# cristian-jfv/lattice-boltzmann-method

Hardware: AMD Instinct MI355X
Metric: MLUPS (million lattice updates/sec), D2Q9 BGK periodic box, f64 (higher is better)
Workload: dtype f64

## Files before the change

### lattice-boltzmann-method_amd/csrc/d2q9.hpp

```cpp
#pragma once
#include <type_traits>
#include <hip/hip_runtime.h>

#include "../../include/lbm_hip.h"

namespace lbm {

constexpr int Q = 9;

#define LBM_W0 (4.0 / 9.0)
#define LBM_WS (1.0 / 9.0)
#define LBM_WD (1.0 / 36.0)

__device__ __forceinline__ constexpr double wq(int q) {
  return q == 0 ? LBM_W0 : (q < 5 ? LBM_WS : LBM_WD);
}
__host__ __device__ __forceinline__ constexpr int icx(int q) {
  return (q == 1 || q == 5 || q == 8) ? 1 : ((q == 3 || q == 6 || q == 7) ? -1 : 0);
}
__host__ __device__ __forceinline__ constexpr int icy(int q) {
  return (q == 2 || q == 5 || q == 6) ? 1 : ((q == 4 || q == 7 || q == 8) ? -1 : 0);
}
__host__ __device__ __forceinline__ constexpr int opp(int q) {
  return q == 0 ? 0 : (q == 1 ? 3 : (q == 2 ? 4 : (q == 3 ? 1 : (q == 4 ? 2 : (q == 5 ? 7 : (q == 6 ? 8 : (q == 7 ? 5 : 6)))))));
// ... 349 lines not shown
    int row_end, int tiles_per_row, double* __restrict__ rho_out, double* __restrict__ u_out) {
  const long items = (long)(row_end - row_begin) * tiles_per_row;
  for (long it = blockIdx.x; it < items; it += gridDim.x) {
    const int r = row_begin + (int)(it / tiles_per_row);
    const int c = (int)(it % tiles_per_row) * 256 + threadIdx.x;
    if (c >= g.C) continue;
    const long rows[3] = {g.at(wrap_row(g, r + 1), 0), g.at(r, 0), g.at(wrap_row(g, r - 1), 0)};
    const int cols[3] = {wrap_col(g, c + 1), c, wrap_col(g, c - 1)};
    double f[Q];
#pragma unroll
    for (int q = 0; q < Q; ++q) {
      const double* src = po + q * g.plane + rows[icx(q) + 1] + cols[icy(q) + 1];
      f[q] = NT_LOAD ? __builtin_nontemporal_load(src) : *src;
    }
    double rho, ux, uy;
    m.collide(f, rho, ux, uy);
#pragma unroll
    for (int q = 0; q < Q; ++q) {
      double* dst = pn + q * g.plane + rows[1] + c;
      if (NT_STORE) __builtin_nontemporal_store(f[q], dst);
      else *dst = f[q];
    }
    if (WITH_MOMENTS) {
      const long o = (long)r * g.C + c, n = (long)g.R * g.C;
      rho_out[o] = rho;
      u_out[o] = ux;
      u_out[n + o] = uy;
    }
  }
}

template <class Model, int BLOCK, int ROWS, bool NT_LOAD, bool NT_STORE>
__global__ __launch_bounds__(BLOCK) void k_stream_collide_v3(
    double* __restrict__ pn, const double* __restrict__ po, Geom g, Model m, int row_begin,
    int row_end, int tiles_x, int n_items, int swizzle) {
  int item = blockIdx.x;
  if (swizzle) {
    const int chunk = (n_items + 7) >> 3;
    item = (item & 7) * chunk + (item >> 3);
    if (item >= n_items) return;
  }
  const int c = (item % tiles_x) * BLOCK + threadIdx.x;
  const int rbase = row_begin + (item / tiles_x) * ROWS;
  if (c >= g.C) return;
  const int cols[3] = {wrap_col(g, c + 1), c, wrap_col(g, c - 1)};
  double f[ROWS][Q];
#pragma unroll
  for (int k = 0; k < ROWS; ++k) {
    const int r = rbase + k;
    if (r < row_end) {
      const long rows[3] = {g.at(wrap_row(g, r + 1), 0), g.at(r, 0), g.at(wrap_row(g, r - 1), 0)};
#pragma unroll
      for (int q = 0; q < Q; ++q) {
        const double* src = po + q * g.plane + rows[icx(q) + 1] + cols[icy(q) + 1];
        f[k][q] = NT_LOAD ? __builtin_nontemporal_load(src) : *src;
      }
    }
  }
#pragma unroll
  for (int k = 0; k < ROWS; ++k) {
    const int r = rbase + k;
    if (r < row_end) {
      double rho, ux, uy;
      m.collide(f[k], rho, ux, uy);
      const long o = g.at(r, c);
#pragma unroll
      for (int q = 0; q < Q; ++q) {
        double* dst = pn + q * g.plane + o;
        if (NT_STORE) __builtin_nontemporal_store(f[k][q], dst);
        else *dst = f[k][q];
      }
    }
  }
}

template <class Model, int TR, int BLOCK, bool NT_STORE>
__global__ __launch_bounds__(BLOCK) void k_stream_collide_tb2(
    double* __restrict__ pn, const double* __restrict__ po, Geom g, Model m, int row_begin,
    int row_end, int tiles_x, int tiles_y, int order) {
  constexpr int TC = 64, LR = TR + 2, LC = TC + 2;
  __shared__ double s[Q][LR][LC];
  int tx, ty;
  if (order == 1) {
    const int xcd = blockIdx.x & 7, j = blockIdx.x >> 3;
    tx = (j / tiles_y) * 8 + xcd;
    ty = j % tiles_y;
  } else {
    tx = blockIdx.x % tiles_x;
    ty = blockIdx.x / tiles_x;
  }
  const int r0 = row_begin + ty * TR, c0 = tx * TC;
  for (int i = threadIdx.x; i < LR * LC; i += BLOCK) {
    const int lr = i / LC, lc = i - lr * LC;
    const int r = wrap_row(g, r0 + lr - 1), c = wrap_col(g, c0 + lc - 1);
    const long rows[3] = {g.at(wrap_row(g, r + 1), 0), g.at(r, 0), g.at(wrap_row(g, r - 1), 0)};
    const int cols[3] = {wrap_col(g, c + 1), c, wrap_col(g, c - 1)};
    double f[Q];
#pragma unroll
    for (int q = 0; q < Q; ++q) f[q] = po[q * g.plane + rows[icx(q) + 1] + cols[icy(q) + 1]];
    double rho, ux, uy;
    m.collide(f, rho, ux, uy);
#pragma unroll
    for (int q = 0; q < Q; ++q) s[q][lr][lc] = f[q];
  }
  __syncthreads();
  for (int i = threadIdx.x; i < TR * TC; i += BLOCK) {
    const int tr = i / TC, tc = i % TC;
    const int r = r0 + tr;
    if (r >= row_end) break;
    double f[Q];
#pragma unroll
    for (int q = 0; q < Q; ++q) f[q] = s[q][tr + 1 - icx(q)][tc + 1 - icy(q)];
    double rho, ux, uy;
    m.collide(f, rho, ux, uy);
    const long o = g.at(r, c0 + tc);
#pragma unroll
    for (int q = 0; q < Q; ++q) {
      double* dst = pn + q * g.plane + o;
      if (NT_STORE) __builtin_nontemporal_store(f[q], dst);
      else *dst = f[q];
    }
  }
}

#ifndef LBM_SW_DPP
#define LBM_SW_DPP 1
#endif
__device__ __forceinline__ double lane_from_prev(double v) {
#if LBM_SW_DPP
  int lo = __double2loint(v), hi = __double2hiint(v);
  lo = __builtin_amdgcn_update_dpp(lo, lo, 0x138, 0xf, 0xf, false);
  hi = __builtin_amdgcn_update_dpp(hi, hi, 0x138, 0xf, 0xf, false);
  return __hiloint2double(hi, lo);
#else
  return __shfl_up(v, 1);
#endif
}
__device__ __forceinline__ double lane_from_next(double v) {
#if LBM_SW_DPP
  int lo = __double2loint(v), hi = __double2hiint(v);
  lo = __builtin_amdgcn_update_dpp(lo, lo, 0x130, 0xf, 0xf, false);
  hi = __builtin_amdgcn_update_dpp(hi, hi, 0x130, 0xf, 0xf, false);
  return __hiloint2double(hi, lo);
#else
  return __shfl_down(v, 1);
#endif
}

constexpr int SW_LDS_LANES = 66;
__host__ __device__ constexpr int sw_lds_level_doubles() { return 12 * SW_LDS_LANES; }
__host__ __device__ constexpr int sw_lds_ring_doubles(int D) { return (D > 1 ? D - 1 : 1) * sw_lds_level_doubles(); }
__host__ __device__ constexpr int sw_grp_pos(int q) { return (q == 3 || q == 0 || q == 1) ? 0 : ((q == 6 || q == 2 || q == 5) ? 1 : 2); }

template <class Model, int D, int K, bool NT_STORE, bool HAS_BC = false, bool LDSR = false>
__device__ __forceinline__ void sw_iteration(double (&ring)[D > 1 ? D - 1 : 1][3][Q], double (&cur)[Q],
                                             double* __restrict__ pn, const double* __restrict__ po,
                                             const Geom& g, const Model& m, int i, int rbase, int R0,
                                             int R1, int c_load, const int (&cols)[3], bool lane_ok,
                                             int c_out, const Bc& bc = Bc{}, int c_raw = 0, double* lds = nullptr, int lane = 0) {
  double nxt[Q];
  {
    const int r1n = rbase + i + 1;
    int rr[3] = {r1n + 1, r1n, r1n - 1};
#pragma unroll
    for (int k = 0; k < 3; ++k) {
      if (g.ghost) rr[k] = rr[k] < -g.ghost ? -g.ghost : (rr[k] > g.R + g.ghost - 1 ? g.R + g.ghost - 1 : rr[k]);
      else rr[k] = rr[k] < 0 ? rr[k] + g.R : (rr[k] >= g.R ? rr[k] - g.R : rr[k]);
    }
#pragma unroll
    for (int q = 0; q < Q; ++q) {
      const char* rowp = reinterpret_cast<const char*>(po + q * g.plane + g.at(rr[icx(q) + 1], 0));
      nxt[q] = *reinterpret_cast<const double*>(rowp + (unsigned)cols[icy(q) + 1] * 8u);
    }
  }
  double f[Q], rho, ux, uy;
#pragma unroll
  for (int q = 0; q < Q; ++q) f[q] = cur[q];
  const bool col_in = c_raw >= 0 && c_raw < g.C;
  const bool wall_col = HAS_BC && col_in && ((c_raw == 0 && bc_is_wall(bc.col_lo)) || (c_raw == g.C - 1 && bc_is_wall(bc.col_hi)));
  const bool rows_wrap = HAS_BC && !g.ghost && !bc_is_wall(bc.row_lo) && !bc_is_wall(bc.row_hi);
  const int row_min = (HAS_BC && g.ghost && bc.row_lo == LBM_EDGE_HALO) ? -g.ghost : 0;
  const int row_max = (HAS_BC && g.ghost && bc.row_hi == LBM_EDGE_HALO) ? g.R + g.ghost - 1 : g.R - 1;
  if (HAS_BC) {
    int r1 = rbase + i;
    if (rows_wrap) r1 = r1 < 0 ? r1 + g.R : (r1 >= g.R ? r1 - g.R : r1);
    const bool wall_row = (r1 == 0 && bc_is_wall(bc.row_lo)) || (r1 == g.R - 1 && bc_is_wall(bc.row_hi));
    if (col_in && r1 >= row_min && r1 <= row_max && (wall_row || wall_col)) gather_walls(f, po, g, bc, r1, c_raw);
  }
  m.collide(f, rho, ux, uy);
#pragma unroll
  for (int l = 2; l <= D; ++l) {
    if constexpr (LDSR) {
      double* lv = lds + (l - 2) * sw_lds_level_doubles();
      double* slotA = lv;
      double* slotB = lv + 3 * SW_LDS_LANES;
      double* slotC = lv + (6 + 3 * (i & 1)) * SW_LDS_LANES;
      double fn[Q];
#pragma unroll
      for (int q = 0; q < Q; ++q) {
        if (icx(q) == 0) fn[q] = slotB[sw_grp_pos(q) * SW_LDS_LANES + lane + 1 - icy(q)];
        else if (icx(q) == 1) fn[q] = slotC[sw_grp_pos(q) * SW_LDS_LANES + lane + 1 - icy(q)];
      }
      __builtin_amdgcn_fence(__ATOMIC_RELEASE, "wavefront");
      __builtin_amdgcn_wave_barrier();
#pragma unroll
      for (int q = 0; q < Q; ++q) {
        double* dst = icx(q) == -1 ? slotA : (icx(q) == 0 ? slotB : slotC);
        dst[sw_grp_pos(q) * SW_LDS_LANES + lane + 1] = f[q];
      }
      __builtin_amdgcn_fence(__ATOMIC_RELEASE, "wavefront");
      __builtin_amdgcn_wave_barrier();
      __builtin_amdgcn_fence(__ATOMIC_ACQUIRE, "wavefront");
#pragma unroll
      for (int q = 0; q < Q; ++q)
        if (icx(q) == -1) fn[q] = slotA[sw_grp_pos(q) * SW_LDS_LANES + lane + 1 - icy(q)];
#pragma unroll
      for (int q = 0; q < Q; ++q) f[q] = fn[q];
    } else {
#pragma unroll
    for (int q = 0; q < Q; ++q) ring[l - 2][K][q] = f[q];
#pragma unroll
    for (int q = 0; q < Q; ++q) {
      const int slot = icx(q) == -1 ? K : (icx(q) == 0 ? (K + 2) % 3 : (K + 1) % 3);
      double v = ring[l - 2][slot][q];
      if (icy(q) == 1) v = lane_from_prev(v);
      else if (icy(q) == -1) v = lane_from_next(v);
      f[q] = v;
    }
    }
    if (HAS_BC && !LDSR) {
      int rl = rbase + i - (l - 1);
      if (rows_wrap) rl = rl < 0 ? rl + g.R : (rl >= g.R ? rl - g.R : rl);
      const bool wall_row = (rl == 0 && bc_is_wall(bc.row_lo)) || (rl == g.R - 1 && bc_is_wall(bc.row_hi));
      if (col_in && rl >= row_min && rl <= row_max && (wall_row || wall_col)) {
        double own[Q];
#pragma unroll
        for (int q = 0; q < Q; ++q) own[q] = ring[l - 2][(K + 2) % 3][q];
        bc_fixups_own(f, own, g, bc, rl, c_raw);
      }
    }
    m.collide(f, rho, ux, uy);
  }
  const int rD = rbase + i - (D - 1);
  if (lane_ok && rD >= R0 && rD < R1) {
    const long o = g.at(rD, 0);
#pragma unroll
    for (int q = 0; q < Q; ++q) {
      double* dst = reinterpret_cast<double*>(reinterpret_cast<char*>(pn + q * g.plane + o) + (unsigned)c_out * 8u);
      if (NT_STORE) __builtin_nontemporal_store(f[q], dst);
      else *dst = f[q];
    }
  }
#pragma unroll
  for (int q = 0; q < Q; ++q) cur[q] = nxt[q];
  (void)c_load;
}

#ifdef LBM_EXPERIMENTS
#include "experiments/sw_prefetch2.hpp"
#endif

__host__ __device__ constexpr int sw_strip_width(int D, bool full = false) {
  return full ? 64 - 2 * (D - 1) : (64 - 2 * (D - 1)) / 8 * 8;
}
template <class M, class = void>
struct sw_full_strips : std::false_type {};
template <class M>
struct sw_full_strips<M, std::void_t<decltype(M::kFullStrips)>> : std::bool_constant<M::kFullStrips> {};
__host__ __device__ constexpr int sw_waves_per_simd(int D) { return D <= 2 ? 4 : (D == 3 ? 3 : (D <= 5 ? 2 : 1)); }
template <class Model, int D, bool NT_STORE, bool HAS_BC, bool PF2, bool LDSR = false>
__device__ __forceinline__ void sw_wave_body(double* __restrict__ pn, const double* __restrict__ po, const Geom& g,
                                             const Model& m, int row_begin, int row_end, int rows_per_chunk, int strips,
                                             int wave, int lane, const Bc& bc, int strip0, int chunk_stride,
                                             double* lds = nullptr) {
  static_assert(!(LDSR && (HAS_BC || PF2)), "the LDS ring exists for the plain window only");
  constexpr int W = sw_strip_width(D, sw_full_strips<Model>::value);
  const int strip = strip0 + wave % strips, chunk = wave / strips;
  const int R0 = row_begin + chunk * (chunk_stride > 0 ? chunk_stride : rows_per_chunk);
  const int R1 = R0 + rows_per_chunk < row_end ? R0 + rows_per_chunk : row_end;
  int c = strip * W - (D - 1) + lane;
  const int c_raw = c;
  const bool lane_ok = lane >= D - 1 && lane < D - 1 + W && c < g.C;
  const bool walled_cols = HAS_BC && (bc_is_wall(bc.col_lo) || bc_is_wall(bc.col_hi));
  if (walled_cols) {
    c = c < 0 ? 0 : (c > g.C - 1 ? g.C - 1 : c);
  } else {
    c = c < 0 ? c + g.C : (c >= g.C ? c - g.C : c);
    c = c >= g.C ? c - g.C : c;
  }
  const int cols[3] = {walled_cols ? (c + 1 > g.C - 1 ? g.C - 1 : c + 1) : wrap_col(g, c + 1), c,
                       walled_cols ? (c - 1 < 0 ? 0 : c - 1) : wrap_col(g, c - 1)};
  const int rbase = R0 - (D - 1);
  const int n_iter = (R1 - R0) + 2 * (D - 1);
  double ring[D > 1 ? D - 1 : 1][3][Q];
#pragma unroll
  for (int a = 0; a < (D > 1 ? D - 1 : 1); ++a)
#pragma unroll
    for (int b = 0; b < 3; ++b)
#pragma unroll
      for (int q = 0; q < Q; ++q) ring[a][b][q] = 1.0;
#ifdef LBM_EXPERIMENTS
  if constexpr (PF2 && !HAS_BC) {
    double raw[3][Q];
#pragma unroll
    for (int a = 0; a < 2; ++a) {
      int rr[3] = {rbase + a + 1, rbase + a, rbase + a - 1};
#pragma unroll
      for (int k = 0; k < 3; ++k) {
        if (g.ghost) rr[k] = rr[k] < -g.ghost ? -g.ghost : (rr[k] > g.R + g.ghost - 1 ? g.R + g.ghost - 1 : rr[k]);
        else rr[k] = rr[k] < 0 ? rr[k] + g.R : (rr[k] >= g.R ? rr[k] - g.R : rr[k]);
      }
#pragma unroll
      for (int q = 0; q < Q; ++q) raw[a][q] = po[q * g.plane + g.at(rr[icx(q) + 1], 0) + cols[icy(q) + 1]];
    }
#pragma unroll
    for (int q = 0; q < Q; ++q) raw[2][q] = 0.0;
    for (int i = 0; i < n_iter; i += 3) {
      sw_iteration_pf2<Model, D, 0, NT_STORE>(ring, raw, pn, po, g, m, i, rbase, R0, R1, cols, lane_ok, c);
      sw_iteration_pf2<Model, D, 1, NT_STORE>(ring, raw, pn, po, g, m, i + 1, rbase, R0, R1, cols, lane_ok, c);
      sw_iteration_pf2<Model, D, 2, NT_STORE>(ring, raw, pn, po, g, m, i + 2, rbase, R0, R1, cols, lane_ok, c);
    }
    return;
  }
#else
  static_assert(!PF2, "the two-row prefetch is an experiment (make EXPERIMENTS=1)");
#endif
  double cur[Q];
  {
    int rr[3] = {rbase + 1, rbase, rbase - 1};
#pragma unroll
    for (int k = 0; k < 3; ++k) {
      if (g.ghost) rr[k] = rr[k] < -g.ghost ? -g.ghost : (rr[k] > g.R + g.ghost - 1 ? g.R + g.ghost - 1 : rr[k]);
      else rr[k] = rr[k] < 0 ? rr[k] + g.R : (rr[k] >= g.R ? rr[k] - g.R : rr[k]);
    }
#pragma unroll
    for (int q = 0; q < Q; ++q) cur[q] = po[q * g.plane + g.at(rr[icx(q) + 1], 0) + cols[icy(q) + 1]];
  }
  const int c_bc = walled_cols ? c_raw : c;
  if constexpr (LDSR) {
    for (int k = lane; k < sw_lds_ring_doubles(D); k += 64) lds[k] = 1.0;
    __builtin_amdgcn_fence(__ATOMIC_RELEASE, "wavefront");
    __builtin_amdgcn_wave_barrier();
    __builtin_amdgcn_fence(__ATOMIC_ACQUIRE, "wavefront");
  }
  for (int i = 0; i < n_iter; i += 3) {
    sw_iteration<Model, D, 0, NT_STORE, HAS_BC, LDSR>(ring, cur, pn, po, g, m, i, rbase, R0, R1, c, cols, lane_ok, c, bc, c_bc, lds, lane);
    sw_iteration<Model, D, 1, NT_STORE, HAS_BC, LDSR>(ring, cur, pn, po, g, m, i + 1, rbase, R0, R1, c, cols, lane_ok, c, bc, c_bc, lds, lane);
    sw_iteration<Model, D, 2, NT_STORE, HAS_BC, LDSR>(ring, cur, pn, po, g, m, i + 2, rbase, R0, R1, c, cols, lane_ok, c, bc, c_bc, lds, lane);
  }
}

template <class Model, int D, int WAVES, bool NT_STORE, bool HAS_BC = false, bool PF2 = false, bool LDSR = false>
__global__ __launch_bounds__(64 * WAVES, (LDSR ? 2 : (WAVES == 4 ? sw_waves_per_simd(D) : 1))) void k_stream_collide_sw(
    double* __restrict__ pn, const double* __restrict__ po, Geom g, Model m, int row_begin,
    int row_end, int rows_per_chunk, int strips, int n_waves, int xcd_group, Bc bc = Bc{}, int strip0 = 0,
    int chunk_stride = 0) {
  int blk = blockIdx.x;
  if (xcd_group > 0) {
    const int x = blk % 8, mth = blk / 8, win = 8 * xcd_group;
    if ((mth / xcd_group + 1) * win <= (int)gridDim.x) blk = (mth / xcd_group) * win + x * xcd_group + mth % xcd_group;
  }
  const int wave = blk * WAVES + __builtin_amdgcn_readfirstlane(threadIdx.x >> 6), lane = threadIdx.x & 63;
  if (wave >= n_waves) return;
  if constexpr (LDSR) {
    __shared__ double lring[WAVES * sw_lds_ring_doubles(D)];
    sw_wave_body<Model, D, NT_STORE, HAS_BC, PF2, true>(pn, po, g, m, row_begin, row_end, rows_per_chunk, strips, wave, lane, bc, strip0, chunk_stride,
                                                        lring + (threadIdx.x >> 6) * sw_lds_ring_doubles(D));
  } else {
    sw_wave_body<Model, D, NT_STORE, HAS_BC, PF2>(pn, po, g, m, row_begin, row_end, rows_per_chunk, strips, wave, lane, bc, strip0, chunk_stride);
  }
}

struct SwPart {
  int r0, r1, s0, ns, rpc, wave0;
};
struct SwParts {
  SwPart p[5];
  int n_frame_waves, n_waves;
};
template <class Model, int D, bool NT_STORE>
__global__ __launch_bounds__(128, 1) void k_stream_collide_sw_walls(double* __restrict__ pn, const double* __restrict__ po,
                                                                    Geom g, Model m, Bc bc, SwParts parts) {
  const int wave = blockIdx.x * 2 + __builtin_amdgcn_readfirstlane(threadIdx.x >> 6), lane = threadIdx.x & 63;
  if (wave >= parts.n_waves) return;
  if (wave < parts.n_frame_waves) {
    int k = 0;
#pragma unroll
    for (int a = 1; a < 4; ++a)
      if (parts.p[a].ns > 0 && parts.p[a].r1 > parts.p[a].r0 && wave >= parts.p[a].wave0) k = a;
    const SwPart pt = parts.p[k];
    sw_wave_body<Model, D, NT_STORE, true, false>(pn, po, g, m, pt.r0, pt.r1, pt.rpc, pt.ns, wave - pt.wave0, lane, bc, pt.s0, 0);
  } else {
    const SwPart pt = parts.p[4];
    sw_wave_body<Model, D, NT_STORE, false, false>(pn, po, g, m, pt.r0, pt.r1, pt.rpc, pt.ns, wave - pt.wave0, lane, bc, pt.s0, 0);
  }
}

#ifdef LBM_EXPERIMENTS
#include "experiments/sw_paired_strips.hpp"
#endif
#ifdef LBM_EXPERIMENTS
#include "experiments/sw_two_columns.hpp"
#endif

template <class Model, bool WITH_MOMENTS>
__global__ __launch_bounds__(256) void k_edge_stream_collide(
    double* __restrict__ pn, const double* __restrict__ po, Geom g, Bc bc, Model m, int row_begin,
    int row_end, double* __restrict__ rho_out, double* __restrict__ u_out) {
  const int i = blockIdx.x * blockDim.x + threadIdx.x, n = row_end - row_begin;
  int r, c;
  if (i < g.C) { r = 0; c = i; }
  else if (i < 2 * g.C) { r = g.R - 1; c = i - g.C; }
  else if (i < 2 * g.C + n) { r = row_begin + i - 2 * g.C; c = 0; }
  else if (i < 2 * g.C + 2 * n) { r = row_begin + i - 2 * g.C - n; c = g.C - 1; }
  else return;
  if (r < row_begin || r >= row_end) return;
  if (i >= 2 * g.C && (r == 0 || r == g.R - 1)) return;
  double f[Q], rho, ux, uy;
  gather_bc(f, po, g, bc, r, c);
  m.collide(f, rho, ux, uy);
  const long o = g.at(r, c);
#pragma unroll
  for (int q = 0; q < Q; ++q) pn[q * g.plane + o] = f[q];
  if (WITH_MOMENTS) {
    const long n = (long)g.R * g.C, oo = (long)r * g.C + c;
    rho_out[oo] = rho;
    u_out[oo] = ux;
    u_out[n + oo] = uy;
  }
}

template <class Model, bool FROM_POST, bool WITH_MOMENTS>
__global__ __launch_bounds__(256) void k_generic_collide(
    double* __restrict__ pn, const double* __restrict__ in, Geom g, Bc bc, Model m, int row_begin,
    int row_end, double* __restrict__ rho_out, double* __restrict__ u_out) {
  const long n_nodes = (long)(row_end - row_begin) * g.C;
  for (long i = (long)blockIdx.x * blockDim.x + threadIdx.x; i < n_nodes;
       i += (long)gridDim.x * blockDim.x) {
    const int r = row_begin + (int)(i / g.C), c = (int)(i % g.C);
    double f[Q], rho, ux, uy;
    if (FROM_POST) {
      gather_bc(f, in, g, bc, r, c);
    } else {
#pragma unroll
      for (int q = 0; q < Q; ++q) f[q] = in[q * g.plane + g.at(r, c)];
    }
    m.collide(f, rho, ux, uy);
    const long o = g.at(r, c);
#pragma unroll
    for (int q = 0; q < Q; ++q) pn[q * g.plane + o] = f[q];
    if (WITH_MOMENTS) {
      const long n = (long)g.R * g.C, oo = (long)r * g.C + c;
      rho_out[oo] = rho;
      u_out[oo] = ux;
      u_out[n + oo] = uy;
    }
  }
}

}
```

### lattice-boltzmann-method_amd/csrc/launch.hpp

```cpp
#pragma once
#include <map>
#include <mutex>
#include <utility>
#include "d2q9.hpp"
#include "internal.hpp"

namespace lbm {

inline int validate_geom_bc(const char* fn, const lbm_geom* g, const lbm_bc* bc, bool reads_neighbours = true) {
  LBM_REQUIRE(g, "%s: NULL geometry", fn);
  LBM_REQUIRE(g->R >= 1 && g->C >= 1, "%s: R=%d C=%d must be positive", fn, g->R, g->C);
  LBM_REQUIRE(g->ghost >= 0 && g->ghost <= 15, "%s: ghost=%d must be 0..15", fn, g->ghost);
  LBM_REQUIRE(g->row_pitch == 0 || (g->row_pitch >= g->C && g->row_pitch % 2 == 0), "%s: row_pitch=%d must be even and >= C=%d (0 = dense)",
              fn, g->row_pitch, g->C);
  LBM_REQUIRE(g->plane_stride == 0 || g->plane_stride >= (long long)(g->R + 2 * g->ghost) * (g->row_pitch > 0 ? g->row_pitch : g->C),
              "%s: plane_stride=%lld smaller than a plane", fn, g->plane_stride);
  if (bc) {
    auto row_ok = [](int m) {
      return m == LBM_EDGE_PERIODIC || m == LBM_EDGE_HALO || m == LBM_EDGE_BOUNCE_BACK ||
             m == LBM_EDGE_ABB_VELOCITY;
    };
    auto col_ok = [](int m) {
      return m == LBM_EDGE_PERIODIC || m == LBM_EDGE_BOUNCE_BACK || m == LBM_EDGE_SPECULAR ||
             m == LBM_EDGE_WRAP_NOSHIFT;
// ... 117 lines not shown
  if (tr == TRV && block == BV) {                                                                 \
    const int tiles_y = (nrows + TRV - 1) / TRV;                                                  \
    const long nblk = (long)tiles_x * tiles_y;                                                    \
    LBM_REQUIRE(nblk < (1L << 30), "%s: lattice too large for one launch", fn);                   \
    if (nt) LBM_KLAUNCH((k_stream_collide_tb2<Model, TRV, BV, true>), dim3((unsigned)nblk), dim3(BV), 0, st, pn, po, g, m, row_begin, row_end, tiles_x, tiles_y, order); \
    else LBM_KLAUNCH((k_stream_collide_tb2<Model, TRV, BV, false>), dim3((unsigned)nblk), dim3(BV), 0, st, pn, po, g, m, row_begin, row_end, tiles_x, tiles_y, order);   \
  } else
  LBM_TB2(4, 256) LBM_TB2(6, 256) LBM_TB2(8, 256) LBM_TB2(8, 512) LBM_TB2(12, 256) LBM_TB2(12, 512)
  LBM_TB2(14, 512) LBM_TB2(16, 512) LBM_TB2(16, 1024) LBM_TB2(30, 1024) {
    set_error("%s: no two-step instantiation for tb_rows=%d tb_block=%d", fn, tr, block);
    return LBM_ERR_INVALID;
  }
#undef LBM_TB2
  LBM_CHECK_LAUNCH();
  return LBM_OK;
}

inline int sw_pick_rows(int nrows, int strips, int depth, long slots) {
  auto cost = [&](int rows) {
    const long waves = (long)strips * ((nrows + rows - 1) / rows);
    const long rounds = (waves + slots - 1) / slots;
    return (double)rounds * (rows + 2 * (depth - 1)) * (1.0 + 0.25 / ((double)rounds * (double)rounds));
  };
  int best = nrows < 64 ? nrows : 64;
  double best_cost = cost(best) * 0.95;
  for (int rows = 32; rows <= 256 && rows <= nrows; rows += 4) {
    const double c = cost(rows);
    if (c < best_cost) best = rows, best_cost = c;
  }
  return best;
}

inline long sw_wave_slots(const void* kernel, int block_threads) {
  static std::mutex mu;
  static std::map<std::pair<const void*, int>, long> cache;
  int dev = 0;
  if (hipGetDevice(&dev) != hipSuccess) {
    (void)hipGetLastError();
    return 0;
  }
  std::lock_guard<std::mutex> lk(mu);
  auto it = cache.find({kernel, dev});
  if (it != cache.end()) return it->second;
  int blocks_per_cu = 0, cus = 0;
  long slots = 0;
  if (hipOccupancyMaxActiveBlocksPerMultiprocessor(&blocks_per_cu, kernel, block_threads, 0) == hipSuccess &&
      hipDeviceGetAttribute(&cus, hipDeviceAttributeMultiprocessorCount, dev) == hipSuccess && blocks_per_cu > 0 && cus > 0)
    slots = (long)blocks_per_cu * (block_threads / 64) * cus;
  else
    (void)hipGetLastError();
  cache[{kernel, dev}] = slots;
  return slots;
}

template <class Model, int DV, bool HAS_BC>
void sw_launch_part(double* pn, const double* po, const Geom& g, const Model& m, const Bc& bc, int r0,
                    int r1, int s0, int ns, int rows_fixed, hipStream_t st) {
  if (r0 >= r1 || ns <= 0) return;
  const int nrows = r1 - r0;
  int rpc = rows_fixed > 0 ? rows_fixed : tuning("sw_rows", -1);
  if (rpc <= 0) {
    const long slots = sw_wave_slots((const void*)k_stream_collide_sw<Model, DV, 2, true, HAS_BC>, 128);
    rpc = slots > 0 ? sw_pick_rows(nrows, ns, DV, slots) : 64;
  }
  if (rpc > nrows) rpc = nrows;
  const int n_waves = ns * ((nrows + rpc - 1) / rpc);
  LBM_KLAUNCH((k_stream_collide_sw<Model, DV, 2, true, HAS_BC>), dim3((n_waves + 1) / 2), dim3(128), 0, st, pn, po, g, m,
              r0, r1, rpc, ns, n_waves, 0, bc, s0);
}

struct SwSideStream {
  hipStream_t st = nullptr;
  hipEvent_t fork = nullptr, join = nullptr;
  int dev = -1;
};
inline SwSideStream* sw_side_stream() {
  static thread_local SwSideStream side[16];
  int dev = 0;
  if (hipGetDevice(&dev) != hipSuccess || dev < 0 || dev >= 16) return nullptr;
  SwSideStream& s = side[dev];
  if (s.dev != dev) {
    if (hipStreamCreateWithFlags(&s.st, hipStreamNonBlocking) != hipSuccess ||
        hipEventCreateWithFlags(&s.fork, hipEventDisableTiming) != hipSuccess ||
        hipEventCreateWithFlags(&s.join, hipEventDisableTiming) != hipSuccess) {
      (void)hipGetLastError();
      return nullptr;
    }
    s.dev = dev;
  }
  return &s;
}

template <class Model, int DV>
int sw_launch_walls(double* pn, const double* po, const Geom& g, const Model& m, const Bc& bc,
                    int row_begin, int row_end, hipStream_t st) {
  constexpr int W = sw_strip_width(DV, sw_full_strips<Model>::value);
  const int strips = (g.C + W - 1) / W;
  const bool col_walls = bc_is_wall(bc.col_lo) || bc_is_wall(bc.col_hi);
  int ra = row_begin, rb = row_end, s0 = 0, s1 = strips;
  if (bc_is_wall(bc.row_lo)) ra = row_begin > 16 ? row_begin : 16;
  if (bc_is_wall(bc.row_hi)) rb = row_end < g.R - 16 ? row_end : g.R - 16;
  if (col_walls) {
    s0 = 1;
    s1 = (g.C - W - DV) / W + 1;
    if (s1 > strips) s1 = strips;
  }
  int split = tuning("sw_split", -1);
  if (split < 0) split = (row_begin == 0 && row_end == g.R && !g.ghost) ? 1 : 2;
  if (split == 0 || ra >= rb || s0 >= s1) {
    sw_launch_part<Model, DV, true>(pn, po, g, m, bc, row_begin, row_end, 0, strips, 0, st);
    return LBM_OK;
  }
  if (split == 2) {
    SwParts pp{};
    const int fr = 8;
    auto part = [&](int k, int r0, int r1, int s0f, int ns, int rpc, int& wave0) {
      if (r1 < r0) r1 = r0;
      if (ns < 0) ns = 0;
      if (rpc > r1 - r0) rpc = r1 - r0;
      pp.p[k] = SwPart{r0, r1, s0f, ns, rpc > 0 ? rpc : 1, wave0};
      if (r1 > r0 && ns > 0) wave0 += ns * ((r1 - r0 + pp.p[k].rpc - 1) / pp.p[k].rpc);
    };
    int w0 = 0;
    part(0, row_begin, row_end, 0, s0, fr, w0);
    part(1, row_begin, row_end, s1, strips - s1, fr, w0);
    part(2, row_begin, ra, s0, s1 - s0, fr, w0);
    part(3, rb, row_end, s0, s1 - s0, fr, w0);
    pp.n_frame_waves = w0;
    int rpc = tuning("sw_rows", -1);
    if (rpc <= 0) {
      const long slots = sw_wave_slots((const void*)k_stream_collide_sw_walls<Model, DV, true>, 128);
      rpc = slots > 0 ? sw_pick_rows(rb - ra, s1 - s0, DV, slots) : 64;
    }
    part(4, ra, rb, s0, s1 - s0, rpc, w0);
    pp.n_waves = w0;
    LBM_KLAUNCH((k_stream_collide_sw_walls<Model, DV, true>), dim3((pp.n_waves + 1) / 2), dim3(128), 0, st, pn, po, g, m, bc, pp);
    return LBM_OK;
  }
  SwSideStream* sd = sw_side_stream();
  hipStream_t fs = st;
  if (sd && hipEventRecord(sd->fork, st) == hipSuccess && hipStreamWaitEvent(sd->st, sd->fork, 0) == hipSuccess) fs = sd->st;
  sw_launch_part<Model, DV, true>(pn, po, g, m, bc, row_begin, row_end, 0, s0, 8, fs);
  sw_launch_part<Model, DV, true>(pn, po, g, m, bc, row_begin, row_end, s1, strips - s1, 8, fs);
  sw_launch_part<Model, DV, true>(pn, po, g, m, bc, row_begin, ra, s0, s1 - s0, 8, fs);
  sw_launch_part<Model, DV, true>(pn, po, g, m, bc, rb, row_end, s0, s1 - s0, 8, fs);
  sw_launch_part<Model, DV, false>(pn, po, g, m, bc, ra, rb, s0, s1 - s0, 0, st);
  if (fs != st) {
    LBM_CHECK_HIP(hipEventRecord(sd->join, fs));
    LBM_CHECK_HIP(hipStreamWaitEvent(st, sd->join, 0));
  }
  return LBM_OK;
}

template <class Model>
int launch_stream_collide_sw(const char* fn, double* pn, const double* po, const lbm_geom* lg,
                             const lbm_bc* lbc, const Model& m, int depth, int row_begin,
                             int row_end, hipStream_t st, int default_waves = 4, int second_begin = -1) {
  if (second_begin >= 0) {
    LBM_REQUIRE(lg && second_begin >= row_end && second_begin + (row_end - row_begin) <= lg->R && row_end - row_begin <= 192,
                "%s: second row range [%d, +%d) must follow the first and fit the lattice", fn, second_begin, row_end - row_begin);
    const Bc b2 = make_bc(lbc);
    if (bc_needs_edge_pass(b2)) {
      int rc2 = launch_stream_collide_sw(fn, pn, po, lg, lbc, m, depth, row_begin, row_end, st, default_waves);
      if (rc2) return rc2;
      return launch_stream_collide_sw(fn, pn, po, lg, lbc, m, depth, second_begin, second_begin + (row_end - row_begin), st, default_waves);
    }
  }
  int rc = validate_geom_bc(fn, lg, lbc);
  if (rc) return rc;
  LBM_REQUIRE(pn && po && pn != po, "%s: NULL or aliased lattices", fn);
  LBM_REQUIRE(0 <= row_begin && row_begin <= row_end && row_end <= lg->R,
              "%s: row range [%d, %d) outside [0, %d)", fn, row_begin, row_end, lg->R);
  const Bc bc = make_bc(lbc);
  auto carried = [](int m) { return m == LBM_EDGE_PERIODIC || m == LBM_EDGE_HALO || bc_is_wall(m); };
  LBM_REQUIRE(carried(bc.row_lo) && carried(bc.row_hi) && carried(bc.col_lo) && carried(bc.col_hi) && !bc.pressure_rows,
              "%s: multi-step launches carry periodic / halo / bounce-back / specular / velocity edges only", fn);
  LBM_REQUIRE(!bc_mixed_axis(bc), "%s: multi-step launches need both edges of an axis walled or neither (wall + PERIODIC on one axis: use single steps)", fn);
  const bool walls = bc_needs_edge_pass(bc);
  LBM_REQUIRE(depth >= 2 && depth <= (walls ? 5 : 6), "%s: %d steps per launch (supported: 2..%d)", fn, depth, walls ? 5 : 6);
  LBM_REQUIRE(lg->ghost == 0 || lg->ghost >= depth, "%s: ghost=%d rows, need 0 or >= %d", fn, lg->ghost, depth);
  LBM_REQUIRE(lg->R >= 4 * depth + 8 && lg->C >= 64, "%s: lattice %dx%d too small for %d-step launches", fn, lg->R, lg->C, depth);
  if (row_begin == row_end) return LBM_OK;
  const Geom g = make_geom(*lg);
  const int nrows = row_end - row_begin;
  const int W = sw_strip_width(depth, sw_full_strips<Model>::value);
  const int strips = (g.C + W - 1) / W;
  LBM_REQUIRE((long)strips * ((nrows + 31) / 32) < (1L << 30), "%s: lattice too large for one launch", fn);
  const int nt = tuning("nt", 3) & 2, waves = tuning("sw_waves", default_waves);
  int rpc = 0, n_waves = 0;
  auto plan = [&](const void* kernel, int block_threads) {
    rpc = tuning("sw_rows", -1);
    if (rpc <= 0) {
      const long slots = sw_wave_slots(kernel, block_threads);
      rpc = slots > 0 ? sw_pick_rows(nrows, strips, depth, slots) : 64;
    }
    if (rpc > nrows) rpc = nrows;
    n_waves = strips * ((nrows + rpc - 1) / rpc);
    if (second_begin >= 0) rpc = nrows, n_waves = 2 * strips;
  };
  const int chunk_stride = second_begin >= 0 ? second_begin - row_begin : 0;
  const int row_end_k = second_begin >= 0 ? second_begin + nrows : row_end;
  if (walls) {
#define LBM_SWBC(DV)                                                                              \
  if (depth == DV) {                                                                              \
    rc = sw_launch_walls<Model, DV>(pn, po, g, m, bc, row_begin, row_end, st);                    \
    if (rc) return rc;                                                                            \
  } else
    LBM_SWBC(2) LBM_SWBC(3) LBM_SWBC(4) LBM_SWBC(5) {
      set_error("%s: no wall-carrying sliding-window instantiation for depth=%d", fn, depth);
      return LBM_ERR_INVALID;
    }
#undef LBM_SWBC
    LBM_CHECK_LAUNCH();
    return LBM_OK;
  }
  bool launched = false;
#ifdef LBM_EXPERIMENTS
  if constexpr (std::is_same<Model, BgkFastModel>::value || std::is_same<Model, BgkModelT<0, 0>>::value) {
    const int pw = tuning("sw_pair", 0);
    if ((pw == 2 || pw == 4) && depth == 5 && nt && g.C >= 256) {
      const int GW = swp_group_width(5, pw), groups = (g.C + GW - 1) / GW;
      int rows = tuning("sw_rows", -1);
      if (second_begin >= 0) rows = nrows;
      else if (rows <= 0) {
        const long slots = pw == 2 ? sw_wave_slots((const void*)k_stream_collide_swp<Model, 5, 2, true>, 128)
                                   : sw_wave_slots((const void*)k_stream_collide_swp<Model, 5, 4, true>, 256);
        rows = slots > 0 ? sw_pick_rows(nrows, groups * pw, 7, slots) : 64;
      }
      if (rows > nrows) rows = nrows;
      const int chunks = second_begin >= 0 ? 2 : (nrows + rows - 1) / rows, total = groups * chunks;
      if (pw == 2) LBM_KLAUNCH((k_stream_collide_swp<Model, 5, 2, true>), dim3(total), dim3(128), 0, st, pn, po, g, m, row_begin, row_end_k, rows, groups, total, chunk_stride);
      else LBM_KLAUNCH((k_stream_collide_swp<Model, 5, 4, true>), dim3(total), dim3(256), 0, st, pn, po, g, m, row_begin, row_end_k, rows, groups, total, chunk_stride);
      launched = true;
    }
  }
  if constexpr (std::is_same<Model, BgkFastModel>::value) {
    if (!launched && tuning("sw_cols2", 0) && (depth == 5 || depth == 6) && nt && g.C % 2 == 0 && g.P % 2 == 0 && g.plane % 2 == 0 &&
        ((uintptr_t)pn % 16) == 0 && ((uintptr_t)po % 16) == 0) {
      const int W2 = sw2_strip_width(depth), strips2 = (g.C + W2 - 1) / W2;
      int rows = tuning("sw_rows", -1);
      const void* kp = depth == 5 ? (const void*)k_stream_collide_sw2<Model, 5, true> : (const void*)k_stream_collide_sw2<Model, 6, true>;
      if (second_begin >= 0) rows = nrows;
      else if (rows <= 0) {
        const long slots = sw_wave_slots(kp, 128);
        rows = slots > 0 ? sw_pick_rows(nrows, strips2, depth, slots) : 64;
      }
      if (rows > nrows) rows = nrows;
      const int nw = second_begin >= 0 ? 2 * strips2 : strips2 * ((nrows + rows - 1) / rows);
      if (depth == 5) LBM_KLAUNCH((k_stream_collide_sw2<Model, 5, true>), dim3((nw + 1) / 2), dim3(128), 0, st, pn, po, g, m, row_begin, row_end_k, rows, strips2, nw, chunk_stride);
      else LBM_KLAUNCH((k_stream_collide_sw2<Model, 6, true>), dim3((nw + 1) / 2), dim3(128), 0, st, pn, po, g, m, row_begin, row_end_k, rows, strips2, nw, chunk_stride);
      launched = true;
    }
  }
  if constexpr (std::is_same<Model, BgkFastModel>::value) {
    if (!launched && tuning("sw_pf2", 0) && depth == 5 && waves == 2 && nt) {
      plan((const void*)k_stream_collide_sw<Model, 5, 2, true, false, true>, 128);
      LBM_KLAUNCH((k_stream_collide_sw<Model, 5, 2, true, false, true>), dim3((n_waves + 1) / 2), dim3(128), 0, st, pn, po, g, m,
                  row_begin, row_end_k, rpc, strips, n_waves, tuning("sw_xcd", 0), Bc{}, 0, chunk_stride);
      launched = true;
    }
  }
#endif
  if (!launched) {
#define LBM_SW(DV, WV)                                                                            \
  if (depth == DV && waves == WV) {                                                               \
    plan((const void*)k_stream_collide_sw<Model, DV, WV, true>, 64 * WV);                         \
    const dim3 grid((n_waves + WV - 1) / WV);                                                     \
    if (nt) LBM_KLAUNCH((k_stream_collide_sw<Model, DV, WV, true>), grid, dim3(64 * WV), 0, st, pn, po, g, m, row_begin, row_end_k, rpc, strips, n_waves, tuning("sw_xcd", 0), Bc{}, 0, chunk_stride); \
    else LBM_KLAUNCH((k_stream_collide_sw<Model, DV, WV, false>), grid, dim3(64 * WV), 0, st, pn, po, g, m, row_begin, row_end_k, rpc, strips, n_waves, tuning("sw_xcd", 0), Bc{}, 0, chunk_stride);   \
  } else
  LBM_SW(2, 4) LBM_SW(3, 4) LBM_SW(4, 4) LBM_SW(5, 4) LBM_SW(6, 4)
  LBM_SW(2, 1) LBM_SW(3, 1) LBM_SW(4, 1) LBM_SW(2, 2) LBM_SW(3, 2) LBM_SW(4, 2) LBM_SW(5, 2) LBM_SW(6, 2) {
    set_error("%s: no sliding-window instantiation for depth=%d sw_waves=%d", fn, depth, waves);
    return LBM_ERR_INVALID;
  }
  }
#undef LBM_SW
  LBM_CHECK_LAUNCH();
  return LBM_OK;
}

template <class Model>
int launch_collide_only(const char* fn, double* p, const double* f, const lbm_geom* lg,
                        const lbm_bc* lbc, const Model& m, double* rho, double* u, hipStream_t st) {
  int rc = validate_geom_bc(fn, lg, lbc, false);
  if (rc) return rc;
  LBM_REQUIRE(p && f, "%s: NULL lattice", fn);
  LBM_REQUIRE((rho == nullptr) == (u == nullptr), "%s: rho and u must both be given or both NULL", fn);
  const Geom g = make_geom(*lg);
  const Bc bc = make_bc(lbc);
  const long n = (long)g.R * g.C;
  const int grid = capped_grid((n + 255) / 256);
  if (rho) LBM_KLAUNCH((k_generic_collide<Model, false, true>), dim3(grid), dim3(256), 0, st, p, f, g, bc, m, 0, g.R, rho, u);
  else LBM_KLAUNCH((k_generic_collide<Model, false, false>), dim3(grid), dim3(256), 0, st, p, f, g, bc, m, 0, g.R, rho, u);
  LBM_CHECK_LAUNCH();
  return LBM_OK;
}

}
```

### lattice-boltzmann-method_amd/pylbm/__init__.py

```python
import ctypes as ct
import os
import re

import numpy as np

_HERE = os.path.dirname(os.path.abspath(__file__))
PKG_DIR = os.path.dirname(_HERE)
REPO = os.path.dirname(PKG_DIR)
LIB_PATH = os.environ.get("LBM_HIP_LIB", os.path.join(PKG_DIR, "lib", "liblbm_hip.so"))
HEADER = os.path.join(REPO, "include", "lbm_hip.h")

EDGE_PERIODIC, EDGE_HALO, EDGE_BOUNCE_BACK, EDGE_SPECULAR, EDGE_ABB_VELOCITY, EDGE_WRAP_NOSHIFT = range(6)
HALO_TWO_PHASE = -3
MODEL_BGK, MODEL_KBC = 0, 1
FORM_DEFAULT, FORM_REFERENCE_ORDER, FORM_REASSOCIATED = 0, 1, 2
RING_DEFAULT, RING_RCCL, RING_IPC = -1, 0, 1
CG_PART_FRAME, CG_PART_INNER = 1, 2
ADE_PART_FRAME, ADE_PART_INNER = 1, 2
ADE_SCALAR_NO_FLUX, ADE_SCALAR_FIXED = 0, 1

_dp = ct.POINTER(ct.c_double)


class Geom(ct.Structure):
    _fields_ = [("R", ct.c_int), ("C", ct.c_int), ("ghost", ct.c_int),
                ("plane_stride", ct.c_longlong), ("row_pitch", ct.c_int)]

    def __init__(self, R=0, C=0, ghost=0, plane_stride=0, row_pitch=0):
        super().__init__(R, C, ghost, plane_stride, row_pitch)


class Bc(ct.Structure):
    _fields_ = [("row_lo", ct.c_int), ("row_hi", ct.c_int), ("col_lo", ct.c_int),
                ("col_hi", ct.c_int), ("pressure_rows", ct.c_int), ("rho_inlet", ct.c_double),
                ("rho_outlet", ct.c_double), ("uw_r", ct.c_double), ("uw_c", ct.c_double)]

    def __init__(self, row_lo=0, row_hi=0, col_lo=0, col_hi=0, pressure_rows=0, rho_inlet=1.0,
                 rho_outlet=1.0, uw_r=0.0, uw_c=0.0):
        super().__init__(row_lo, row_hi, col_lo, col_hi, pressure_rows, rho_inlet, rho_outlet, uw_r, uw_c)

    @staticmethod
    def periodic():
        return Bc()


class BgkParams(ct.Structure):
    _fields_ = [("omega", ct.c_double), ("incompressible", ct.c_int), ("delta_form", ct.c_int),
                ("force_mode", ct.c_int), ("force_r", ct.c_double), ("force_c", ct.c_double),
                ("guo_a", ct.c_double), ("guo_b", ct.c_double), ("form", ct.c_int)]

    def __init__(self, omega=1.0, incompressible=0, delta_form=0, force=None, guo=(1.0 / 3.0, 1.0 / 9.0), form=FORM_DEFAULT):
        if force is None:
            super().__init__(omega, incompressible, delta_form, 0, 0.0, 0.0, 0.0, 0.0, form)
        else:
            super().__init__(omega, incompressible, 1, 1, force[0], force[1], guo[0], guo[1], form)


class KbcParams(ct.Structure):
    _fields_ = [("s2", ct.c_double), ("form", ct.c_int)]

    def __init__(self, s2=1.0, form=FORM_DEFAULT):
        super().__init__(s2, form)


class CgColour(ct.Structure):
    _fields_ = [("rho_0", ct.c_double), ("alpha", ct.c_double), ("nu", ct.c_double),
                ("beta", ct.c_double)]


class CgParams(ct.Structure):
    _fields_ = [("red", CgColour), ("blue", CgColour), ("sigma", ct.c_double),
                ("gravity_r", ct.c_double), ("gravity_c", ct.c_double), ("add_source", ct.c_int),
                ("delta", ct.c_double), ("form", ct.c_int)]


class AdeParams(ct.Structure):
    _fields_ = [("omega_g", ct.c_double), ("w_r", ct.c_double), ("w_c", ct.c_double), ("form", ct.c_int)]

    def __init__(self, omega_g=1.0, w=(0.0, 0.0), form=FORM_DEFAULT):
        super().__init__(omega_g, w[0], w[1], form)


class AdeScalarBC(ct.Structure):
    EDGES = ("row_lo", "row_hi", "col_lo", "col_hi")
    _fields_ = [("mode", ct.c_int * 4), ("conc", ct.c_double * 4), ("profile", _dp * 4)]

    def __init__(self, **fixed):
        super().__init__()
        self._keep = []
        for name, v in fixed.items():
            e = self.EDGES.index(name)
            conc, prof = (v if isinstance(v, tuple) else (v, None))
            self.mode[e] = ADE_SCALAR_FIXED
            self.conc[e] = float(conc)
            self.profile[e] = _ptr(prof) if prof is not None else ct.cast(None, _dp)
            if prof is not None and not isinstance(prof, int):
                self._keep.append(prof)


class LbmError(RuntimeError):
    pass


def declared_symbols(header=HEADER):
    txt = open(header).read()
    txt = re.sub(r"/\*.*?\*/", "", txt, flags=re.S)
    return sorted(set(re.findall(r"\b(lbm_[a-z0-9_]+)\s*\(", txt)))


def load_library(path=LIB_PATH):
    if not os.path.exists(path):
        raise LbmError(
            f"{path} not found: build it with `python -c 'import __graft_entry__ as g; g.build()'` "
            "or `make -C lattice-boltzmann-method_amd/csrc` (no CPU fallback exists)")
    lib = ct.CDLL(path)
    lib.lbm_last_error_string.restype = ct.c_char_p
    lib.lbm_default_plane_pad.restype = ct.c_longlong
    lib.lbm_solver_block_launches.restype = ct.c_longlong
    lib.lbm_slab_ibm_msg_doubles.restype = ct.c_longlong
    lib.lbm_cg_solver_pair_launches.restype = ct.c_longlong
    lib.lbm_slab_pressure_msg_doubles.restype = ct.c_longlong
    lib.lbm_ade_solver_launches.restype = ct.c_longlong
    return lib


class Lib:

    def __init__(self, path=LIB_PATH):
        self.raw = load_library(path)

    def __getattr__(self, name):
        fn = getattr(self.raw, "lbm_" + name)

        def call(*args):
            rc = fn(*args)
            if rc != 0:
                raise LbmError(f"lbm_{name} -> {rc}: {self.raw.lbm_last_error_string().decode()}")
            return rc

        return call

    def device_count(self):
        return self.raw.lbm_device_count()

    def default_plane_pad(self, R, C):
        return int(self.raw.lbm_default_plane_pad(R, C))

    def reset_tuning(self):
        for k in (b"variant", b"nt", b"grid_cap", b"block", b"rows", b"xcd_swizzle", b"tb_rows", b"tb_block", b"tb_order", b"sw_rows", b"sw_waves", b"solver_depth", b"cg_fused", b"cg_tile", b"cg_xcd", b"kbc_fast", b"kbc_depth", b"bgk_fast", b"cg_strip", b"cg_rows", b"cg_split", b"sw_split", b"solver_depth_walls", b"ibm_depth", b"ibm_gate", b"bgk_fast_delta", b"pressure_depth", b"halo_grid", b"cg_strip2", b"cg_rows2", b"sw_pair", b"sw_pf2", b"cg_strip_xcd", b"cg_merge", b"cg_frame_beside", b"ring_period", b"ibm_step_opt", b"ibm_step_split", b"ibm_step_chain", b"ibm_box", b"ibm_box_overlap", b"bg_priority", b"ibm_chain_kernel", b"ibm_chain_wgs", b"ibm_box_sole", b"sw_ldsring", b"ring_ipc_timeout_ms", b"cg_big", b"cg_big_xcd", b"ring_ipc_force_cached", b"ring_ipc_cached_ok", b"row_pad", b"cg_walk_rows", b"cg_walk_tile_xcd", b"sw_cols2"):
            self.set_tuning(k, -1)


def _ptr(t):
    if t is None:
        return ct.cast(None, _dp)
    if isinstance(t, int):
        return ct.cast(t, _dp)
    assert t.stride(-1) == 1 and str(t.dtype) == "torch.float64", (t.dtype, t.stride())
    return ct.cast(t.data_ptr(), _dp)


def _hptr(a):
    assert a.dtype == np.float64 and a.flags["C_CONTIGUOUS"]
    return a.ctypes.data_as(_dp)


def _stream(s):
    return ct.c_void_p(0 if s is None else int(s))


class Solver:

    def __init__(self, lib, model, R, C, params, bc=None, stream=None):
        self.lib, self.R, self.C = lib, R, C
        self.g = Geom(R, C, 0)
        self.bc = bc if bc is not None else Bc.periodic()
        self.params = params
        self.h = ct.c_void_p()
        lib.solver_create(ct.byref(self.h), model, ct.byref(self.g), ct.byref(self.bc),
                          ct.byref(params), _stream(stream))

    def close(self):
        if self.h:
            self.lib.solver_destroy(self.h)
            self.h = ct.c_void_p()

    def __del__(self):
        try:
            self.close()
        except Exception:
            pass

    def set_f(self, f):
        f = np.ascontiguousarray(f, dtype=np.float64)
        assert f.shape == (self.R, self.C, 9)
        self.lib.solver_set_f_aos(self.h, _hptr(f))

    def set_moments(self, rho, u):
        rho = np.ascontiguousarray(rho, dtype=np.float64)
        u = np.ascontiguousarray(u, dtype=np.float64)
        assert rho.shape == (self.R, self.C) and u.shape == (self.R, self.C, 2)
        self.lib.solver_set_moments_aos(self.h, _hptr(rho), _hptr(u))

    def get_f(self):
        f = np.empty((self.R, self.C, 9))
        self.lib.solver_get_f_aos(self.h, _hptr(f))
        return f

    def step(self, n, record_moments=False):
        self.lib.solver_step(self.h, int(n), int(bool(record_moments)))

    def moments(self):
        rho = np.empty((self.R, self.C))
        u = np.empty((self.R, self.C, 2))
        self.lib.solver_get_moments_aos(self.h, _hptr(rho), _hptr(u))
        return rho, u

    def sync(self):
        self.lib.solver_sync(self.h)

    def checkpoint_save(self, path):
        self.lib.solver_checkpoint_save(self.h, str(path).encode())

    def checkpoint_load(self, path):
        self.lib.solver_checkpoint_load(self.h, str(path).encode())

    def attach_ibm(self, ibm, guo_a=1.0 / 3.0, guo_b=1.0 / 9.0):
        self._ibm = ibm
        self.lib.solver_attach_ibm(self.h, ibm.h, ct.c_double(guo_a), ct.c_double(guo_b))

    def lattices(self):
        a, b, g = _dp(), _dp(), Geom()
        self.lib.solver_lattices(self.h, ct.byref(a), ct.byref(b), ct.byref(g))
        return ct.cast(a, ct.c_void_p).value, ct.cast(b, ct.c_void_p).value, g


class AdeSolver:

    def __init__(self, lib, R, C, fluid, scalar, bc=None, stream=None, scalar_bc=None):
        self.lib, self.R, self.C, self.fluid, self.scalar = lib, R, C, fluid, scalar
        self.g = Geom(R, C, 0)
        self.bc = bc if bc is not None else Bc.periodic()
        self.h = ct.c_void_p()
        lib.ade_solver_create(ct.byref(self.h), ct.byref(self.g), ct.byref(self.bc), ct.byref(fluid),
                              ct.byref(scalar), _stream(stream))
        self.scalar_bc = None
        if scalar_bc is not None:
            try:
                self.set_scalar_bc(scalar_bc)
            except LbmError:
                self.close()
                raise

    def set_scalar_bc(self, scalar_bc):
        self.lib.ade_solver_set_scalar_bc(self.h, ct.byref(scalar_bc) if scalar_bc is not None else None)
        self.scalar_bc = scalar_bc

    def close(self):
        if self.h:
            self.lib.ade_solver_destroy(self.h)
            self.h = ct.c_void_p()

    def __del__(self):
        try:
            self.close()
        except Exception:
            pass

    def set_state(self, f, g):
        f = np.ascontiguousarray(f, dtype=np.float64)
        g = np.ascontiguousarray(g, dtype=np.float64)
        assert f.shape == (self.R, self.C, 9) and g.shape == (self.R, self.C, 9)
        self.lib.ade_solver_set_state(self.h, _hptr(f), _hptr(g))

    def step(self, n):
        self.lib.ade_solver_step(self.h, int(n))

    def get_state(self):
        R, C = self.R, self.C
        out = dict(f=np.empty((R, C, 9)), g=np.empty((R, C, 9)), rho=np.empty((R, C)), u=np.empty((R, C, 2)),
                   C=np.empty((R, C)))
        self.lib.ade_solver_get_state(self.h, *[_hptr(out[k]) for k in ("f", "g", "rho", "u", "C")])
        return out

    def sync(self):
        self.lib.ade_solver_sync(self.h)

    def launches(self):
        return int(self.lib.raw.lbm_ade_solver_launches(self.h))

    def lattices(self):
        p = [_dp() for _ in range(4)]
        g = Geom()
        self.lib.ade_solver_lattices(self.h, *[ct.byref(x) for x in p], ct.byref(g))
        return tuple(ct.cast(x, ct.c_void_p).value for x in p) + (g,)


def cg_params(red=(3.0, 0.7, 0.04, 0.7), blue=(1.0, 0.1, 0.04, -0.7), sigma=0.1, gravity=6.25e-6,
              delta=0.1, gravity_c=0.0, add_source=1, form=FORM_DEFAULT):
    return CgParams(CgColour(*red), CgColour(*blue), sigma, gravity, gravity_c, add_source, delta, form)


# ... 106 lines not shown
```

Baseline: 173,400.

## Run adjacent sliding-window strips as lockstep groups with per-row barriers

```diff
diff --git a/lattice-boltzmann-method_amd/csrc/d2q9.hpp b/lattice-boltzmann-method_amd/csrc/d2q9.hpp
--- a/lattice-boltzmann-method_amd/csrc/d2q9.hpp
+++ b/lattice-boltzmann-method_amd/csrc/d2q9.hpp
@@ -525,12 +525,13 @@
 __host__ __device__ constexpr int sw_lds_ring_doubles(int D) { return (D > 1 ? D - 1 : 1) * sw_lds_level_doubles(); }
 __host__ __device__ constexpr int sw_grp_pos(int q) { return (q == 3 || q == 0 || q == 1) ? 0 : ((q == 6 || q == 2 || q == 5) ? 1 : 2); }
 
-template <class Model, int D, int K, bool NT_STORE, bool HAS_BC = false, bool LDSR = false>
+template <class Model, int D, int K, bool NT_STORE, bool HAS_BC = false, bool LDSR = false, bool LOCKSTEP = false>
 __device__ __forceinline__ void sw_iteration(double (&ring)[D > 1 ? D - 1 : 1][3][Q], double (&cur)[Q],
                                              double* __restrict__ pn, const double* __restrict__ po,
                                              const Geom& g, const Model& m, int i, int rbase, int R0,
                                              int R1, int c_load, const int (&cols)[3], bool lane_ok,
                                              int c_out, const Bc& bc = Bc{}, int c_raw = 0, double* lds = nullptr, int lane = 0) {
+  if constexpr (LOCKSTEP) __builtin_amdgcn_s_barrier();
   double nxt[Q];
   {
     const int r1n = rbase + i + 1;
@@ -641,12 +642,13 @@
 template <class M>
 struct sw_full_strips<M, std::void_t<decltype(M::kFullStrips)>> : std::bool_constant<M::kFullStrips> {};
 __host__ __device__ constexpr int sw_waves_per_simd(int D) { return D <= 2 ? 4 : (D == 3 ? 3 : (D <= 5 ? 2 : 1)); }
-template <class Model, int D, bool NT_STORE, bool HAS_BC, bool PF2, bool LDSR = false>
+template <class Model, int D, bool NT_STORE, bool HAS_BC, bool PF2, bool LDSR = false, bool LOCKSTEP = false>
 __device__ __forceinline__ void sw_wave_body(double* __restrict__ pn, const double* __restrict__ po, const Geom& g,
                                              const Model& m, int row_begin, int row_end, int rows_per_chunk, int strips,
                                              int wave, int lane, const Bc& bc, int strip0, int chunk_stride,
                                              double* lds = nullptr) {
   static_assert(!(LDSR && (HAS_BC || PF2)), "the LDS ring exists for the plain window only");
+  static_assert(!(LOCKSTEP && (HAS_BC || PF2 || LDSR)), "strip groups in lockstep exist for the plain register window only");
   constexpr int W = sw_strip_width(D, sw_full_strips<Model>::value);
   const int strip = strip0 + wave % strips, chunk = wave / strips;
   const int R0 = row_begin + chunk * (chunk_stride > 0 ? chunk_stride : rows_per_chunk);
@@ -717,9 +719,9 @@
     __builtin_amdgcn_fence(__ATOMIC_ACQUIRE, "wavefront");
   }
   for (int i = 0; i < n_iter; i += 3) {
-    sw_iteration<Model, D, 0, NT_STORE, HAS_BC, LDSR>(ring, cur, pn, po, g, m, i, rbase, R0, R1, c, cols, lane_ok, c, bc, c_bc, lds, lane);
-    sw_iteration<Model, D, 1, NT_STORE, HAS_BC, LDSR>(ring, cur, pn, po, g, m, i + 1, rbase, R0, R1, c, cols, lane_ok, c, bc, c_bc, lds, lane);
-    sw_iteration<Model, D, 2, NT_STORE, HAS_BC, LDSR>(ring, cur, pn, po, g, m, i + 2, rbase, R0, R1, c, cols, lane_ok, c, bc, c_bc, lds, lane);
+    sw_iteration<Model, D, 0, NT_STORE, HAS_BC, LDSR, LOCKSTEP>(ring, cur, pn, po, g, m, i, rbase, R0, R1, c, cols, lane_ok, c, bc, c_bc, lds, lane);
+    sw_iteration<Model, D, 1, NT_STORE, HAS_BC, LDSR, LOCKSTEP>(ring, cur, pn, po, g, m, i + 1, rbase, R0, R1, c, cols, lane_ok, c, bc, c_bc, lds, lane);
+    sw_iteration<Model, D, 2, NT_STORE, HAS_BC, LDSR, LOCKSTEP>(ring, cur, pn, po, g, m, i + 2, rbase, R0, R1, c, cols, lane_ok, c, bc, c_bc, lds, lane);
   }
 }
 
@@ -742,6 +744,17 @@
   } else {
     sw_wave_body<Model, D, NT_STORE, HAS_BC, PF2>(pn, po, g, m, row_begin, row_end, rows_per_chunk, strips, wave, lane, bc, strip0, chunk_stride);
   }
+}
+
+template <class Model, int D, int G, bool NT_STORE>
+__global__ __launch_bounds__(64 * G, 1) void k_stream_collide_swg(double* __restrict__ pn, const double* __restrict__ po, Geom g, Model m,
+                                                                  int row_begin, int row_end, int rows_per_chunk, int strips,
+                                                                  int groups, int chunk_stride) {
+  const int w = __builtin_amdgcn_readfirstlane(threadIdx.x >> 6), lane = threadIdx.x & 63;
+  const int strip = ((int)blockIdx.x % groups) * G + w, chunk = (int)blockIdx.x / groups;
+  if (strip >= strips) return;
+  sw_wave_body<Model, D, NT_STORE, false, false, false, true>(pn, po, g, m, row_begin, row_end, rows_per_chunk, strips, chunk * strips + strip,
+                                                              lane, Bc{}, 0, chunk_stride);
 }
 
 struct SwPart {
diff --git a/lattice-boltzmann-method_amd/csrc/launch.hpp b/lattice-boltzmann-method_amd/csrc/launch.hpp
--- a/lattice-boltzmann-method_amd/csrc/launch.hpp
+++ b/lattice-boltzmann-method_amd/csrc/launch.hpp
@@ -293,6 +293,26 @@
   return LBM_OK;
 }
 
+constexpr int kSwGroupDefault = 4;
+template <class Model, int SG>
+void sw_launch_group(double* pn, const double* po, const Geom& g, const Model& m, int row_begin, int row_end, int second_begin,
+                     int strips, bool nt, hipStream_t st) {
+  const int nrows = row_end - row_begin, groups = (strips + SG - 1) / SG;
+  const void* kernel = nt ? (const void*)k_stream_collide_swg<Model, 5, SG, true> : (const void*)k_stream_collide_swg<Model, 5, SG, false>;
+  int rpc = tuning("sw_rows", -1);
+  if (rpc <= 0) {
+    const long slots = sw_wave_slots(kernel, 64 * SG);
+    rpc = slots > 0 ? sw_pick_rows(nrows, groups * SG, 5, slots) : 64;
+  }
+  if (rpc > nrows || second_begin >= 0) rpc = nrows;
+  const int chunks = second_begin >= 0 ? 2 : (nrows + rpc - 1) / rpc;
+  const int chunk_stride = second_begin >= 0 ? second_begin - row_begin : 0;
+  const int row_end_k = second_begin >= 0 ? second_begin + nrows : row_end;
+  const dim3 grid((unsigned)(groups * chunks));
+  if (nt) LBM_KLAUNCH((k_stream_collide_swg<Model, 5, SG, true>), grid, dim3(64 * SG), 0, st, pn, po, g, m, row_begin, row_end_k, rpc, strips, groups, chunk_stride);
+  else LBM_KLAUNCH((k_stream_collide_swg<Model, 5, SG, false>), grid, dim3(64 * SG), 0, st, pn, po, g, m, row_begin, row_end_k, rpc, strips, groups, chunk_stride);
+}
+
 template <class Model>
 int launch_stream_collide_sw(const char* fn, double* pn, const double* po, const lbm_geom* lg,
                              const lbm_bc* lbc, const Model& m, int depth, int row_begin,
@@ -402,6 +422,15 @@
     }
   }
 #endif
+  if constexpr (std::is_same<Model, BgkFastModel>::value || std::is_same<Model, BgkModelT<0, 0>>::value) {
+    const bool dflt = std::is_same<Model, BgkFastModel>::value && strips >= kSwGroupDefault && tuning("sw_waves", -1) < 0;
+    const int grp = depth == 5 && !launched ? tuning("sw_group", dflt ? kSwGroupDefault : 0) : 0;
+    if (grp == 4) sw_launch_group<Model, 4>(pn, po, g, m, row_begin, row_end, second_begin, strips, nt != 0, st), launched = true;
+    else if (grp != 0) {
+      set_error("%s: no strip-group instantiation for sw_group=%d (supported: 0, 4)", fn, grp);
+      return LBM_ERR_INVALID;
+    }
+  }
   if (!launched) {
 #define LBM_SW(DV, WV)                                                                            \
   if (depth == DV && waves == WV) {                                                               \
diff --git a/lattice-boltzmann-method_amd/pylbm/__init__.py b/lattice-boltzmann-method_amd/pylbm/__init__.py
--- a/lattice-boltzmann-method_amd/pylbm/__init__.py
+++ b/lattice-boltzmann-method_amd/pylbm/__init__.py
@@ -147,7 +147,7 @@
         return int(self.raw.lbm_default_plane_pad(R, C))
 
     def reset_tuning(self):
-        for k in (b"variant", b"nt", b"grid_cap", b"block", b"rows", b"xcd_swizzle", b"tb_rows", b"tb_block", b"tb_order", b"sw_rows", b"sw_waves", b"solver_depth", b"cg_fused", b"cg_tile", b"cg_xcd", b"kbc_fast", b"kbc_depth", b"bgk_fast", b"cg_strip", b"cg_rows", b"cg_split", b"sw_split", b"solver_depth_walls", b"ibm_depth", b"ibm_gate", b"bgk_fast_delta", b"pressure_depth", b"halo_grid", b"cg_strip2", b"cg_rows2", b"sw_pair", b"sw_pf2", b"cg_strip_xcd", b"cg_merge", b"cg_frame_beside", b"ring_period", b"ibm_step_opt", b"ibm_step_split", b"ibm_step_chain", b"ibm_box", b"ibm_box_overlap", b"bg_priority", b"ibm_chain_kernel", b"ibm_chain_wgs", b"ibm_box_sole", b"sw_ldsring", b"ring_ipc_timeout_ms", b"cg_big", b"cg_big_xcd", b"ring_ipc_force_cached", b"ring_ipc_cached_ok", b"row_pad", b"cg_walk_rows", b"cg_walk_tile_xcd", b"sw_cols2"):
+        for k in (b"variant", b"nt", b"grid_cap", b"block", b"rows", b"xcd_swizzle", b"tb_rows", b"tb_block", b"tb_order", b"sw_rows", b"sw_waves", b"sw_group", b"solver_depth", b"cg_fused", b"cg_tile", b"cg_xcd", b"kbc_fast", b"kbc_depth", b"bgk_fast", b"cg_strip", b"cg_rows", b"cg_split", b"sw_split", b"solver_depth_walls", b"ibm_depth", b"ibm_gate", b"bgk_fast_delta", b"pressure_depth", b"halo_grid", b"cg_strip2", b"cg_rows2", b"sw_pair", b"sw_pf2", b"cg_strip_xcd", b"cg_merge", b"cg_frame_beside", b"ring_period", b"ibm_step_opt", b"ibm_step_split", b"ibm_step_chain", b"ibm_box", b"ibm_box_overlap", b"bg_priority", b"ibm_chain_kernel", b"ibm_chain_wgs", b"ibm_box_sole", b"sw_ldsring", b"ring_ipc_timeout_ms", b"cg_big", b"cg_big_xcd", b"ring_ipc_force_cached", b"ring_ipc_cached_ok", b"row_pad", b"cg_walk_rows", b"cg_walk_tile_xcd", b"sw_cols2"):
             self.set_tuning(k, -1)
 
 
```

Measured after the change: 168,100. -3.1%, worse.
